# zssjh/stereo-semantic-vo

Measured on AMD Instinct MI355X. Metric: stereo frames/sec on KITTI 00 (full Tracking::Track chain), higher is better.
Workload: dtype u8; 1 GPU; BASELINE configs[2]: synth-kitti00 sequence of 4541 distinct 1241x376 stereo pairs, full Tracking::Track loop per frame (ORB on L and R, sparse stereo, matching passes 1+2, PnP-RANSAC, pose-only LM, map-point lifecycle); ONE sequence per GPU in strict frame order (replicas across GPUs); parallelism=one GPU, resident_pairs_per_gpu=4541, resident_input_bytes_per_gpu=4370984960, frames_tracked=4541, tracker_capacity_flag=0, pnp_samples_through_sequential_fallback=0

## Files before the change

include/svo.h:

```cpp
#ifndef SVO_H
#define SVO_H

#include <stdint.h>

#ifdef __cplusplus
extern "C" {
#endif

#define SVO_ABI_VERSION 8

typedef enum svo_status {
  SVO_OK = 0,
  SVO_E_INVALID = -1,
  SVO_E_NODEVICE = -2,
  SVO_E_NOMEM = -3,
  SVO_E_HIP = -4,
  SVO_E_CAPACITY = -5,
  SVO_E_TIMEOUT = -6
} svo_status;

typedef struct svo_ctx svo_ctx;

typedef struct svo_kp {
  float x, y;
// ... 87 lines not shown
int svo_orb_extract(svo_ctx* ctx, const uint8_t* gray, int stride, svo_kp* kp,
                    uint8_t* desc, int32_t* n);

int svo_debug_pyramid_level(svo_ctx* ctx, int image_slot, int level, uint8_t* out);
int svo_debug_fast_corners(svo_ctx* ctx, int image_slot, int level, int32_t* xy_score,
                           int capacity, int32_t* n);

int svo_stereo_frame(svo_ctx* ctx, const uint8_t* grayL, int strideL, const uint8_t* grayR,
                     int strideR, const svo_camera* cam, svo_kp* kpL, uint8_t* descL,
                     int32_t* nL, float* uR, float* depth);
int svo_stereo_frame_ex(svo_ctx* ctx, const uint8_t* grayL, int strideL, const uint8_t* grayR,
                        int strideR, const svo_camera* cam, svo_kp* kpL, uint8_t* descL,
                        int32_t* nL, float* uR, float* depth, svo_kp* kpR, uint8_t* descR,
                        int32_t* nR);

int svo_debug_stereo_match(svo_ctx* ctx, const uint8_t* grayL, int strideL, const uint8_t* grayR, int strideR,
                           const svo_camera* cam, const svo_kp* kpL, const uint8_t* descL, int nL, const svo_kp* kpR,
                           const uint8_t* descR, int nR, float* uR, float* depth, int32_t* sad);

int svo_disp2depth(svo_ctx* ctx, const float* disp, int count, float bf, float* depth);
int svo_unproject(svo_ctx* ctx, const float* uvz, int n, const svo_camera* cam,
                  const float Rwc[9], const float twc[3], float* xyz);


int svo_descriptor_distance(svo_ctx* ctx, const uint8_t* a, const uint8_t* b, int count,
                            int32_t* dist);

int svo_hamming_argmin(svo_ctx* ctx, const uint8_t* q, int M, const uint8_t* t, int N,
                       const uint8_t* t_mask, int32_t* best_idx, int32_t* best,
                       int32_t* second);

int svo_match_greedy(svo_ctx* ctx, const uint8_t* q, const uint8_t* q_skip, int M,
                     const uint8_t* t, int N, uint8_t* assigned, int max_dist, float ratio,
                     int32_t* best_idx, int32_t* best, int32_t* second, uint8_t* accepted);

int svo_match_greedy_gated(svo_ctx* ctx, const uint8_t* q, const uint8_t* q_skip, int M,
                           const uint8_t* t, int N, uint8_t* assigned, int max_dist, float ratio,
                           const float* q_xy, const float* t_xy, const int32_t* boxes, int n_boxes,
                           const double F[9], int32_t* best_idx, int32_t* best, int32_t* second,
                           uint8_t* accepted, uint8_t* vetoed);

int svo_bf_match(svo_ctx* ctx, const uint8_t* q, int M, const uint8_t* t, int N,
                 int32_t* train_idx, int32_t* dist, uint8_t* keep);

int svo_fundamental_8point(svo_ctx* ctx, const double* pts1, const double* pts2, int n, double F[9]);

int svo_pnp_ransac(svo_ctx* ctx, const double* Xw, const double* obs, int n, const double K[4],
                   const double T_fallback_cw[16], uint64_t rng_state, double T_cw[16],
                   uint8_t* inlier_mask, svo_pnp_stats* stats);

int svo_debug_epnp5(svo_ctx* ctx, const double Xw5[15], const double uv5[10], const double K[4], double R[9],
                    double t[3], double rep_err[3]);

int svo_pose_opt(svo_ctx* ctx, const double* Xw, const double* obs, int n, const double K[4],
                 double T_cw[16], svo_lm_stats* stats);

int svo_track_reset(svo_ctx* ctx, const svo_camera* cam);
int svo_track_frame(svo_ctx* ctx, const uint8_t* grayL, int strideL, const uint8_t* grayR,
                    int strideR, double timestamp, const int32_t* boxes, int n_boxes,
                    svo_track_result* res);

int svo_debug_track_matches(svo_ctx* ctx, int32_t* cur_mp);
int svo_debug_track_gate(svo_ctx* ctx, double F[9], int32_t* n_vetoed);
int svo_debug_track_frames(svo_ctx* ctx, int first, int n, svo_track_debug* out);

int svo_debug_track_depths(svo_ctx* ctx, int frame, svo_kp* kp, float* depth, int32_t* n);

int svo_debug_track_pnp(svo_ctx* ctx, svo_pnp_stats* stats, double T_pnp[16]);

int svo_frontend_batch_dev(svo_ctx* ctx, const uint8_t* d_grayL, const uint8_t* d_grayR,
                           int stride, int B, const svo_camera* cam, svo_kp* d_kpL,
                           uint8_t* d_descL, int32_t* d_nL, float* d_uR, float* d_depth);
int svo_track_batch_dev(svo_ctx* ctx, const uint8_t* d_grayL, const uint8_t* d_grayR,
                        int stride, int B, const svo_boxes_dev* boxes, svo_track_result* d_results);

int svo_track_tail_dev(svo_ctx* ctx, const svo_kp* d_kp, const uint8_t* d_desc, const int32_t* d_n,
                       const float* d_depth, int kp_stride, int B, const svo_boxes_dev* boxes,
                       svo_track_result* d_results);
int svo_track_sharded_dev(svo_ctx* const* ctxs, int G, const uint8_t* const* d_grayL, const uint8_t* const* d_grayR,
                          int stride, int B, const svo_boxes_dev* boxes, svo_track_result* d_results);
int svo_track_batch_host(svo_ctx* ctx, const uint8_t* grayL, const uint8_t* grayR, int stride, int B,
                         const svo_boxes_host* boxes, svo_track_result* results);
int svo_track_sharded_host(svo_ctx* const* ctxs, int G, const uint8_t* grayL, const uint8_t* grayR, int stride, int B,
                           const svo_boxes_host* boxes, svo_track_result* results);
int svo_frontend_batch_host(svo_ctx* ctx, const uint8_t* grayL, const uint8_t* grayR, int stride, int B,
                            const svo_camera* cam, svo_kp* kpL, uint8_t* descL, int32_t* nL, float* uR, float* depth);


int svo_bgr_to_gray(svo_ctx* ctx, const uint8_t* bgr, int width, int height, int bgr_stride, uint8_t* gray, int gray_stride);
int svo_track_frame_bgr(svo_ctx* ctx, const uint8_t* bgrL, int strideL, const uint8_t* bgrR, int strideR, double timestamp,
                        const int32_t* boxes, int n_boxes, svo_track_result* res);
int svo_track_batch_bgr_dev(svo_ctx* ctx, const uint8_t* d_bgrL, const uint8_t* d_bgrR, int stride, int B,
                            const svo_boxes_dev* boxes, svo_track_result* d_results);
int svo_track_batch_bgr_host(svo_ctx* ctx, const uint8_t* bgrL, const uint8_t* bgrR, int stride, int B,
                             const svo_boxes_host* boxes, svo_track_result* results);

int svo_track_overflowed(svo_ctx* ctx, int32_t* flag);
int svo_track_epnp_fallbacks(svo_ctx* ctx, int64_t* count);

int svo_debug_stream_probe(svo_ctx* ctx, int32_t out[2]);

int svo_debug_stream_pipes(svo_ctx* ctx, int32_t out[4]);

int svo_track_multi_reset(svo_ctx* ctx, int n_seq, const svo_camera* cam);
int svo_track_multi_step_dev(svo_ctx* ctx, const uint8_t* d_grayL, const uint8_t* d_grayR, int stride,
                             int n_seq, const svo_boxes_dev* boxes, svo_track_result* d_results);
// ... 203 lines not shown
```

stereo-semantic-vo_amd/__init__.py:

```python
import ctypes as C
import os

import numpy as np

_HERE = os.path.dirname(os.path.abspath(__file__))
LIB_PATH = os.environ.get("SVO_LIB_PATH") or os.path.join(_HERE, "libsvo_hip.so")

KP_DTYPE = np.dtype([("x", "<f4"), ("y", "<f4"), ("size", "<f4"), ("angle", "<f4"),
                     ("response", "<f4"), ("octave", "<i4"), ("class_id", "<i4")])

TRACK_DTYPE = np.dtype([("Tcw", "<f4", (16,)), ("frame_id", "<i4"), ("n_kp", "<i4"),
                        ("n_stereo", "<i4"), ("n_match_pass1", "<i4"), ("n_match_pass2", "<i4"),
                        ("n_pnp_inliers", "<i4"), ("n_lm_edges", "<i4"), ("n_new_mappoints", "<i4"),
                        ("n_local_map", "<i4"), ("lm_iterations", "<i4"), ("reserved", "<i4", (2,))])

TRACK_DEBUG_DTYPE = np.dtype([("match_gid", "<i4", (512,)), ("new_gid", "<i4", (512,)), ("frame_id", "<i4"),
                              ("pnp_best", "<i4"), ("pnp_iterations", "<i4"), ("pnp_inliers", "<i4"), ("pnp_ok", "<i4"),
                              ("active_rows", "<i4", (2,)), ("rounds", "<i4", (2,)), ("resolve_us", "<i4"),
                              ("rt", "<i8", (6,)), ("T_pnp", "<f8", (16,))])

ABI_SYMBOLS = [
    "svo_abi_version", "svo_strerror", "svo_last_error", "svo_create", "svo_destroy", "svo_sync",
    "svo_set_option",
    "svo_stream", "svo_orb_geometry", "svo_orb_extract", "svo_debug_pyramid_level",
    "svo_debug_fast_corners", "svo_stereo_frame", "svo_stereo_frame_ex", "svo_disp2depth",
    "svo_unproject", "svo_descriptor_distance", "svo_hamming_argmin", "svo_match_greedy",
    "svo_match_greedy_gated",
    "svo_bf_match", "svo_pnp_ransac", "svo_debug_epnp5", "svo_pose_opt", "svo_track_reset", "svo_track_frame",
    "svo_debug_track_matches", "svo_debug_track_gate", "svo_debug_track_pnp", "svo_debug_track_frames", "svo_fundamental_8point",
    "svo_frontend_batch_dev", "svo_track_batch_dev", "svo_profile_enable", "svo_profile_reset",
    "svo_profile_get",
    "svo_elas_default_params", "svo_elas_process", "svo_elas_process_ex", "svo_elas_delaunay",
    "svo_ctmf", "svo_track_multi_reset", "svo_track_multi_step_dev", "svo_track_tail_dev", "svo_track_overflowed", "svo_track_epnp_fallbacks", "svo_debug_stream_probe", "svo_debug_stream_pipes", "svo_track_sharded_dev", "svo_elas_batch_dev", "svo_msa_init", "svo_msa_tree", "svo_msa_tree_dp", "svo_msa_wta", "svo_msa_lrcheck", "svo_msa_solve", "svo_msa_batch_dev",
    "svo_create_ex", "svo_stream_mode", "svo_track_batch_host", "svo_track_sharded_host", "svo_frontend_batch_host",
    "svo_bgr_to_gray", "svo_track_frame_bgr", "svo_track_batch_bgr_dev", "svo_track_batch_bgr_host",
    "svo_det_describe", "svo_det_last_error", "svo_det_create", "svo_det_destroy", "svo_det_detect", "svo_det_batch_dev",
    "svo_det_sync", "svo_det_debug_tensor", "svo_det_detect_planar", "svo_det_profile", "svo_det_layer_times",
    "svo_sgbm_default_params", "svo_sgbm_process", "svo_sgbm_batch_dev", "svo_sgbm_debug_volume", "svo_sgbm_filter_speckles",
    "svo_sgbm_default_params_bgr", "svo_sgbm_process_bgr", "svo_sgbm_batch_bgr_dev", "svo_debug_track_depths",
    "svo_sgbm_process_mode", "svo_sgbm_process_bgr_mode", "svo_sgbm_batch_mode_dev", "svo_sgbm_batch_bgr_mode_dev",
    "svo_lk_default_params", "svo_lk_track", "svo_lk_batch_dev", "svo_lk_chain_dev", "svo_lk_debug_level",
    "svo_lk_track_bgr", "svo_lk_batch_bgr_dev", "svo_lk_chain_bgr_dev", "svo_lk_debug_level_bgr",
    "svo_dyn_default_params", "svo_track_dynamic", "svo_track_dynamic_out", "svo_track_multi_step_bgr_dev",
    "svo_debug_stereo_match",
]

CREATE_POOLED_STREAMS = 1
CREATE_TAIL_ALL_CUS = 2


class SvoError(RuntimeError):
    pass


class Camera(C.Structure):
    _fields_ = [("fx", C.c_float), ("fy", C.c_float), ("cx", C.c_float), ("cy", C.c_float),
                ("bf", C.c_float)]


class BoxesDev(C.Structure):
    _fields_ = [("boxes", C.c_void_p), ("n", C.c_void_p), ("stride", C.c_int32)]


def boxes_dev(d_boxes, d_n, stride):
    return BoxesDev(C.c_void_p(int(d_boxes)), C.c_void_p(int(d_n)), int(stride))


def _bx(b):
    return None if b is None else C.byref(b)


class BoxesHost(C.Structure):
    _fields_ = [("boxes", C.c_void_p), ("n", C.c_void_p), ("stride", C.c_int32)]


def boxes_host(boxes, n):
    b = np.ascontiguousarray(boxes, np.int32)
    c = np.ascontiguousarray(n, np.int32)
    r = BoxesHost(b.ctypes.data_as(C.c_void_p), c.ctypes.data_as(C.c_void_p), int(b.shape[1]))
    r._keep = (b, c)
    return r
# ... 202 lines not shown
        sk = None if q_skip is None else _u8(q_skip)
        bi = np.zeros(M, np.int32); b = np.zeros(M, np.int32); s = np.zeros(M, np.int32)
        acc = np.zeros(M, np.uint8)
        self._chk(self.lib.svo_match_greedy(self.h, _p(q), _p(sk), M, _p(t), N, _p(assigned),
                                            int(max_dist), C.c_float(ratio), _p(bi), _p(b), _p(s),
                                            _p(acc)))
        return bi, b, s, acc, assigned

    def match_greedy_gated(self, q, t, assigned, max_dist, ratio, q_xy, t_xy, boxes, F, q_skip=None, vetoed=None):
        q = _u8(q).reshape(-1, 32); t = _u8(t).reshape(-1, 32)
        M, N = len(q), len(t)
        assigned = _u8(assigned).copy()
        sk = None if q_skip is None else _u8(q_skip)
        qxy = np.ascontiguousarray(q_xy, np.float32).reshape(-1, 2)
        txy = np.ascontiguousarray(t_xy, np.float32).reshape(-1, 2)
        if len(qxy) != M or len(txy) != N:
            raise SvoError("match_greedy_gated: q_xy / t_xy must hold one point per descriptor row")
        bx = None if boxes is None or len(boxes) == 0 else np.ascontiguousarray(boxes, np.int32).reshape(-1, 4)
        nb = 0 if bx is None else len(bx)
        Fm = np.ascontiguousarray(F, np.float64).reshape(9)
        bi = np.zeros(M, np.int32); b = np.zeros(M, np.int32); s = np.zeros(M, np.int32)
        acc = np.zeros(M, np.uint8)
        vet = np.zeros(M, np.uint8) if vetoed is None else vetoed
        if vet.dtype != np.uint8 or vet.shape != (M,) or not vet.flags.c_contiguous:
            raise SvoError("match_greedy_gated: vetoed must be a contiguous uint8 array of M entries")
        self._chk(self.lib.svo_match_greedy_gated(self.h, _p(q), _p(sk), M, _p(t), N, _p(assigned), int(max_dist),
                                                  C.c_float(ratio), _p(qxy), _p(txy), _p(bx), nb, _p(Fm), _p(bi), _p(b),
                                                  _p(s), _p(acc), _p(vet)))
        return bi, b, s, acc, assigned, vet

    def bf_match(self, q, t):
        q = _u8(q).reshape(-1, 32); t = _u8(t).reshape(-1, 32)
        M, N = len(q), len(t)
        ti = np.zeros(M, np.int32); d = np.zeros(M, np.int32); keep = np.zeros(M, np.uint8)
        self._chk(self.lib.svo_bf_match(self.h, _p(q), M, _p(t), N, _p(ti), _p(d), _p(keep)))
        return ti, d, keep

    def pnp_ransac(self, Xw, obs, K, T_fallback, rng_state=0):
        Xw = np.ascontiguousarray(Xw, np.float64).reshape(-1, 3)
        obs = np.ascontiguousarray(obs, np.float64).reshape(-1, 2)
        K = np.ascontiguousarray(K, np.float64)
        Tp = np.ascontiguousarray(T_fallback, np.float64).reshape(16)
        T = np.zeros(16); mask = np.zeros(max(len(Xw), 1), np.uint8); st = PnpStats()
        self._chk(self.lib.svo_pnp_ransac(self.h, _p(Xw), _p(obs), len(Xw), _p(K), _p(Tp),
                                          C.c_uint64(rng_state), _p(T), _p(mask), C.byref(st)))
        return T.reshape(4, 4), mask[:len(Xw)], st

    def debug_epnp5(self, Xw5, uv5, K):
        Xw5 = np.ascontiguousarray(Xw5, np.float64).reshape(15); uv5 = np.ascontiguousarray(uv5, np.float64).reshape(10)
        K = np.ascontiguousarray(K, np.float64); R = np.zeros(9); t = np.zeros(3); rep = np.zeros(3)
        self._chk(self.lib.svo_debug_epnp5(self.h, _p(Xw5), _p(uv5), _p(K), _p(R), _p(t), _p(rep)))
        return R.reshape(3, 3), t, rep

    def pose_opt(self, Xw, obs, K, T):
        Xw = np.ascontiguousarray(Xw, np.float64).reshape(-1, 3)
        obs = np.ascontiguousarray(obs, np.float64).reshape(-1, 2)
        K = np.ascontiguousarray(K, np.float64)
        T = np.ascontiguousarray(T, np.float64).reshape(16).copy()
        st = LmStats()
        self._chk(self.lib.svo_pose_opt(self.h, _p(Xw), _p(obs), len(Xw), _p(K), _p(T), C.byref(st)))
        return T.reshape(4, 4), st

    def track_reset(self, cam):
        self._chk(self.lib.svo_track_reset(self.h, C.byref(cam)))

    def track_frame(self, grayL, grayR, timestamp=0.0, boxes=None):
        grayL = _u8(grayL); grayR = _u8(grayR)
        res = np.zeros(1, TRACK_DTYPE)
        bx = None if boxes is None or len(boxes) == 0 else np.ascontiguousarray(boxes, np.int32)
        nb = 0 if bx is None else len(bx)
        self._chk(self.lib.svo_track_frame(self.h, _p(grayL), self.W, _p(grayR), self.W,
                                           C.c_double(timestamp), _p(bx), nb, _p(res)))
        return res[0]

    def bgr_to_gray(self, bgr):
        a = _u8(bgr)
        H, W = a.shape[:2]
        out = np.zeros((H, W), np.uint8)
        self._chk(self.lib.svo_bgr_to_gray(self.h, _p(a), W, H, 3 * W, _p(out), W))
        return out

    def track_frame_bgr(self, bgrL, bgrR, timestamp=0.0, boxes=None):
        bgrL = _u8(bgrL); bgrR = _u8(bgrR)
        res = np.zeros(1, TRACK_DTYPE)
        bx = None if boxes is None or len(boxes) == 0 else np.ascontiguousarray(boxes, np.int32)
        nb = 0 if bx is None else len(bx)
        self._chk(self.lib.svo_track_frame_bgr(self.h, _p(bgrL), 3 * self.W, _p(bgrR), 3 * self.W,
                                               C.c_double(timestamp), _p(bx), nb, _p(res)))
        return res[0]

    def track_batch_bgr_dev(self, d_bgrL, d_bgrR, stride, B, d_results, boxes=None):
        self._chk(self.lib.svo_track_batch_bgr_dev(self.h, _p(d_bgrL), _p(d_bgrR), int(stride), int(B), _bx(boxes),
                                                   _p(d_results)))

    def track_batch_bgr_host(self, bgrL, bgrR, stride, B, results, boxes=None):
        self._chk(self.lib.svo_track_batch_bgr_host(self.h, _p(bgrL), _p(bgrR), int(stride), int(B), _bx(boxes), _p(results)))

    def debug_track_gate(self):
        F = np.zeros(9); n = C.c_int32(0)
        self._chk(self.lib.svo_debug_track_gate(self.h, _p(F), C.byref(n)))
        return F.reshape(3, 3), n.value

    def fundamental_8point(self, pts1, pts2):
        pts1 = np.ascontiguousarray(pts1, np.float64).reshape(-1, 2)
        pts2 = np.ascontiguousarray(pts2, np.float64).reshape(-1, 2)
        F = np.zeros(9)
# ... 526 lines not shown
```

stereo-semantic-vo_amd/csrc/svo_api.hip:

```cpp
#include <math.h>
#include <string.h>

#include <algorithm>
#include <thread>
#include <stdio.h>
#include <stdlib.h>

#include <chrono>
#include <functional>
#include <initializer_list>
#include "svo_internal.h"

struct PendingEvt { int entry; hipEvent_t a, b; };

struct SvoProfState {
  std::vector<PendingEvt> pending;
  std::vector<hipEvent_t> pool;
};
static SvoProfState* prof_state(svo_ctx* ctx) {
  if (!ctx->prof_impl) ctx->prof_impl = new SvoProfState();
  return reinterpret_cast<SvoProfState*>(ctx->prof_impl);
}
static void prof_resolve(svo_ctx* ctx) {
  SvoProfState* ps = prof_state(ctx);
// ... 810 lines not shown
  hipSetDevice(ctx->device);
  Bump bm{ctx};
  double* dX = bm.take<double>(3 * (size_t)std::max(n, 1));
  double* dO = bm.take<double>(2 * (size_t)std::max(n, 1));
  double* dK = bm.take<double>(4);
  double* dTp = bm.take<double>(16);
  double* dT = bm.take<double>(16);
  uint8_t* dM = bm.take<uint8_t>(std::max(n, 1));
  svo_pnp_stats* dS = bm.take<svo_pnp_stats>(1);
  uint16_t* dSub = bm.take<uint16_t>(512);
  void* dHyp = bm.take<uint8_t>(svo_pnp_hyp_bytes());
  if (!bm.ok()) return SVO_E_CAPACITY;
  if (n > 0) { H2D(dX, Xw, 24 * (size_t)n); H2D(dO, obs, 16 * (size_t)n); }
  H2D(dK, K, 32);
  H2D(dTp, T_fallback_cw, 128);
  const uint16_t* sub = ctx->d_pnp_subsets + (size_t)std::min(n, 512) * 500;
  uint16_t hsub[500];
  if (rng_state != 0 && rng_state != ~0ull) {
    svo_pnp_subsets(rng_state, n, hsub);
    H2D(dSub, hsub, sizeof hsub);
    SVO_HIP(ctx, hipStreamSynchronize(ctx->stream));
    sub = dSub;
  }
  int rc = svo_launch_pnp(ctx, dX, dO, n, dK, dTp, sub, dHyp, dT, dM, dS);
  if (rc) return rc;
  D2H(T_cw, dT, 128);
  if (inlier_mask && n > 0) D2H(inlier_mask, dM, n);
  if (stats) D2H(stats, dS, sizeof(svo_pnp_stats));
  SVO_HIP(ctx, hipStreamSynchronize(ctx->stream));
  return SVO_OK;
}

extern "C" int svo_debug_epnp5(svo_ctx* ctx, const double Xw5[15], const double uv5[10], const double K[4], double R[9],
                               double t[3], double rep_err[3]) {
  if (!ctx || !Xw5 || !uv5 || !K || !R || !t) return SVO_E_INVALID;
  hipSetDevice(ctx->device);
  Bump bm{ctx};
  double* dX = bm.take<double>(15); double* dU = bm.take<double>(10); double* dK = bm.take<double>(4);
  double* dO = bm.take<double>(24);
  if (!bm.ok()) return SVO_E_CAPACITY;
  H2D(dX, Xw5, 120); H2D(dU, uv5, 80); H2D(dK, K, 32);
  const char* reps_env = getenv("SVO_EPNP_REPS");
  int rc = svo_launch_epnp5_probe(ctx, dX, dU, dK, dO, reps_env ? atoi(reps_env) : 1);
  if (rc) return rc;
  double o[24];
  D2H(o, dO, sizeof o);
  SVO_HIP(ctx, hipStreamSynchronize(ctx->stream));
  memcpy(R, o, 72); memcpy(t, o + 9, 24);
  if (rep_err) memcpy(rep_err, o + 13, 24);
  if (getenv("SVO_EPNP_STAMPS")) fprintf(stderr, "epnp5 cycles: setup+MtM %.0f, eigen %.0f (%d sweeps), L/rho %.0f, branches %.0f (initial betas %.0f, Gauss-Newton %.0f, to the last SVD %.0f)\n", o[16], o[17], (int)o[20], o[18], o[19], o[21], o[22], o[23]);
  return o[12] != 0.0 ? SVO_OK : SVO_E_INVALID;
}

static int frontend_slice(svo_ctx* ctx, hipStream_t st, const uint8_t* d_grayL, const uint8_t* d_grayR, int stride, int p0, int b,
                          const svo_camera* cam, svo_kp* d_kpL, uint8_t* d_descL, int32_t* d_nL, float* d_uR, float* d_depth) {
  const size_t K = ctx->max_kp, img = (size_t)ctx->g.H * stride;
  const SvoFeBufs fb = svo_fe_own(ctx).at(ctx->g, K, 2 * (size_t)p0, p0);
  int rc = svo_launch_orb(ctx, st, fb, d_grayL + p0 * img, d_grayR + p0 * img, stride, b, 2 * b);
  if (rc == SVO_OK) rc = svo_launch_stereo(ctx, st, fb, d_grayL + p0 * img, d_grayR + p0 * img, stride, b, cam);
  if (rc == SVO_OK) {
    auto d2d = [&](void* dst, const void* src, size_t bytes) {
      if (dst && hipMemcpyAsync(dst, src, bytes, hipMemcpyDeviceToDevice, st) != hipSuccess) rc = SVO_E_HIP;
    };
    d2d(d_kpL ? d_kpL + (size_t)p0 * K : nullptr, fb.kp, sizeof(svo_kp) * K * b);
    d2d(d_descL ? d_descL + (size_t)p0 * K * 32 : nullptr, fb.desc, 32 * K * b);
    d2d(d_nL ? d_nL + p0 : nullptr, fb.nkp, 4 * (size_t)b);
    d2d(d_uR ? d_uR + (size_t)p0 * K : nullptr, fb.uR, 4 * K * b);
    d2d(d_depth ? d_depth + (size_t)p0 * K : nullptr, fb.depth, 4 * K * b);
  }
  return rc;
}

int svo_frontend_nslices(const svo_ctx* ctx, int B) {
  const int ns = std::min(ctx->opt_frontend_overlap, B / 8);
  return (ns < 2 || ctx->profiling) ? 1 : ns;
}

extern "C" int svo_frontend_batch_dev(svo_ctx* ctx, const uint8_t* d_grayL, const uint8_t* d_grayR,
                                      int stride, int B, const svo_camera* cam, svo_kp* d_kpL,
                                      uint8_t* d_descL, int32_t* d_nL, float* d_uR,
                                      float* d_depth) {
  if (!ctx || !d_grayL || !d_grayR || !cam || B < 1 || stride < ctx->g.W) return SVO_E_INVALID;
  if (B > ctx->max_batch) return SVO_E_CAPACITY;
  hipSetDevice(ctx->device);
  { const int rcq = svo_track_quiesce(ctx); if (rcq) return rcq; }
  const int ns = svo_frontend_nslices(ctx, B);
  if (ns < 2)
    return frontend_slice(ctx, ctx->stream, d_grayL, d_grayR, stride, 0, B, cam, d_kpL, d_descL, d_nL, d_uR, d_depth);
  while ((int)ctx->fe_streams.size() < ns - 1) {
    hipStream_t st = nullptr;
    hipEvent_t e;
    {
      int attempts = 0, percent = 0;
      const int rcp = svo_pick_stream(ctx, [](hipStream_t* s) { return svo_stream_create(s, 0); },
                                      {ctx->stream, ctx->fe_streams.empty() ? nullptr : ctx->fe_streams.back()}, &st, &attempts, &percent,
                                      {ctx->stream, ctx->fe_streams.empty() ? nullptr : ctx->fe_streams.back()},
                                      {ctx->stream, ctx->fe_streams.empty() ? nullptr : ctx->fe_streams.back()});
      if (rcp) return rcp;
    }
    ctx->fe_streams.push_back(st);
    SVO_HIP(ctx, hipEventCreateWithFlags(&e, hipEventDisableTiming));
    ctx->fe_events.push_back(e);
  }
  if (!ctx->ev_frontend) SVO_HIP(ctx, hipEventCreateWithFlags(&ctx->ev_frontend, hipEventDisableTiming));
  SVO_HIP(ctx, hipEventRecord(ctx->ev_frontend, ctx->stream));
  int rc = SVO_OK;
// ... 223 lines not shown
```

stereo-semantic-vo_amd/csrc/svo_epnp_ord_dev.h:

```cpp
#pragma once
#ifndef HIP_INCLUDE_HIP_HIP_RUNTIME_H
#include <hip/hip_runtime.h>
#endif
#include <stdint.h>

#include "svo_epnp_exact_dev.h"

namespace epnp_ord {

#define EO_FN __device__ __forceinline__
typedef double d2 __attribute__((ext_vector_type(2)));

#include "svo_epnp_ord_tab.h"
#include "svo_epnp_ord_asm.h"

#define EO_SYNC()                                         \
  do {                                                    \
    __builtin_amdgcn_fence(__ATOMIC_ACQ_REL, "wavefront"); \
    __builtin_amdgcn_wave_barrier();                      \
  } while (0)

struct Lds {
  alignas(16) double jr[16 * 16];
  alignas(16) double xch[16][4][4];
// ... 377 lines not shown
        const double delta = (gamma - beta) * 0.5;
        sn = xsqrt(xdiv(delta, gamma));
        c = xdiv(p, gamma * sn * 2);
      } else {
        c = xsqrt(xdiv(gamma + beta, gamma * 2));
        sn = xdiv(p, gamma * c * 2);
      }
      const double se = is_j ? -sn : sn;
      const double n0 = c * x0 + se * y0, n1 = c * x1 + se * y1, n2 = c * x2 + se * y2;
      const double Wn = colsum<12>(n0 * n0, n1 * n1, n2 * n2, g);
      EO_SYNC();
      if (rot) {
        x0 = n0; x1 = n1; x2 = n2; W = Wn;
        chg |= 1u << sw;
        mine[0] = x0; mine[1] = x1; mine[2] = x2;
        S.xw[r] = W;
      }
    }
    EO_SYNC();
    const bool closes = active && (e & 0x80u) != 0;
    if (__any(closes)) {
      const int sc = sbase + (int)((e >> 8) & 3);
      const unsigned long long bal = __ballot(closes && ((chg >> (sc & 31)) & 1u));
      if (closes && (sc >= 29 || ((unsigned)bal & pm) == 0u)) active = false;
    }
    tt = tn; tp = tpn; sbase = sbn; e = en;
    ++nsteps;
  }
  if (lane == 0) S.sweeps = 1000000 + nsteps;
  EO_SYNC();
}

typedef __attribute__((address_space(3))) double lds_double;
__device__ __attribute__((noinline)) void svd_small_seq(Lds& S, double* jW, int M, int n, int base, int p) {
  double w[6];
  epnp_exact::jacobi_svd((lds_double*)jW, (lds_double*)&S.jr[base * 16], 16, w, (lds_double*)&S.jr[base * 16 + M], 16, M, n, n);
  for (int i = 0; i < n; ++i) {
    S.sw[p][i] = w[i];
    S.srow[p][i] = base + i;
    S.jr[(base + i) * 16 + 15] = w[i];
  }
  S.flag |= 2; S.why |= 8;
}

__device__ __attribute__((noinline)) void svd12_finish_seq(Lds& S, epnp_exact::Work& xw) {
  for (int i = 0; i < 12; ++i)
    for (int k = 0; k < 12; ++k) xw.ut[i * 12 + k] = S.xch[i][k & 3][k >> 2];
  epnp_exact::jacobi_svd_finish((lds_double*)xw.jW, (lds_double*)xw.ut, 12, xw.d, (lds_double*)nullptr, 0, 12, 12, 12);
  for (int q = 0; q < 4; ++q)
    for (int k = 0; k < 12; ++k) S.ut4[q][k] = xw.ut[(11 - q) * 12 + k];
  S.flag |= 2; S.why |= 4;
}

EO_FN void gauss_newton(Lds& S, int cand, int col, bool owner, const double* L, const double* rho, double* betas) {
  for (int it = 0; it < 5; ++it) {
    double A[6][4], b[6];
    {
      const int i = col < 6 ? col : 0;
      const double* rl = L + 10 * i;
      double* g = S.gn[cand][i];
      const double a0 = 2 * rl[0] * betas[0] + rl[1] * betas[1] + rl[3] * betas[2] + rl[6] * betas[3];
      const double a1 = rl[1] * betas[0] + 2 * rl[2] * betas[1] + rl[4] * betas[2] + rl[7] * betas[3];
      const double a2 = rl[3] * betas[0] + rl[4] * betas[1] + 2 * rl[5] * betas[2] + rl[8] * betas[3];
      const double a3 = rl[6] * betas[0] + rl[7] * betas[1] + rl[8] * betas[2] + 2 * rl[9] * betas[3];
      const double bi = rho[i] - (rl[0] * betas[0] * betas[0] + rl[1] * betas[0] * betas[1] + rl[2] * betas[1] * betas[1] +
                                  rl[3] * betas[0] * betas[2] + rl[4] * betas[1] * betas[2] + rl[5] * betas[2] * betas[2] +
                                  rl[6] * betas[0] * betas[3] + rl[7] * betas[1] * betas[3] + rl[8] * betas[2] * betas[3] +
                                  rl[9] * betas[3] * betas[3]);
      if (owner && col < 6) { g[0] = a0; g[1] = a1; g[2] = a2; g[3] = a3; g[4] = bi; }
    }
    EO_SYNC();
#pragma unroll
    for (int i = 0; i < 6; ++i) {
      const double* g = S.gn[cand][i];
      A[i][0] = g[0]; A[i][1] = g[1]; A[i][2] = g[2]; A[i][3] = g[3]; b[i] = g[4];
    }
    EO_SYNC();
    double A1[4], A2[4], x[4] = {0, 0, 0, 0};
    bool alive = true;
#pragma unroll
    for (int k = 0; k < 4; ++k) {
      double eta = fabs(A[k][k]);
#pragma unroll
      for (int i = k + 1; i < 6; ++i) {
        const double elt = fabs(A[i - 1][k]);
        if (eta < elt) eta = elt;
      }
      if (eta == 0) alive = false;
      const double inv_eta = 1. / eta;
      double sum2 = 0.0;
#pragma unroll
      for (int i = k; i < 6; ++i) {
        A[i][k] *= inv_eta;
        sum2 += A[i][k] * A[i][k];
      }
      double sigma = xsqrt(sum2);
      if (A[k][k] < 0) sigma = -sigma;
      A[k][k] += sigma;
      A1[k] = sigma * A[k][k];
      A2[k] = -eta * sigma;
#pragma unroll
      for (int j = k + 1; j < 4; ++j) {
        double sum = 0;
#pragma unroll
        for (int i = k; i < 6; ++i) sum += A[i][k] * A[i][j];
        const double tau = sum / A1[k];
#pragma unroll
        for (int i = k; i < 6; ++i) A[i][j] -= tau * A[i][k];
      }
    }
#pragma unroll
    for (int j = 0; j < 4; ++j) {
      double tau = 0;
#pragma unroll
      for (int i = j; i < 6; ++i) tau += A[i][j] * b[i];
      tau /= A1[j];
#pragma unroll
      for (int i = j; i < 6; ++i) b[i] -= tau * A[i][j];
    }
    x[3] = b[3] / A2[3];
#pragma unroll
    for (int i = 2; i >= 0; --i) {
      double sum = 0;
#pragma unroll
      for (int j = i + 1; j < 4; ++j) sum += A[i][j] * x[j];
      x[i] = (b[i] - sum) / A2[i];
    }
#pragma unroll
    for (int i = 0; i < 4; ++i) betas[i] += alive ? x[i] : 0.0;
  }
}

EO_FN double dot3(const double* a, const double* b) { return a[0] * b[0] + a[1] * b[1] + a[2] * b[2]; }

EO_FN bool solve5_wave(Lds& S, epnp_exact::Work& xw, const double* K, double* R_out, double* t_out, double* rep, bool force_seq = false) {
  const int lane = threadIdx.x & 63, slot = lane >> 4, col = lane & 15, r16 = lane & 15;
  const double fu = K[0], fv = K[1], uc = K[2], vc = K[3];
  if (lane == 0) { S.flag = force_seq ? 1 : 0; S.why = force_seq ? 16 : 0; S.stamp[0] = clock64(); }
  load_tables(S, lane);
  EO_SYNC();
  if (lane < 3) {
    double c = 0;
    for (int i = 0; i < 5; i++) c += S.pws[3 * i + lane];
    S.cws[lane] = c / 5;
  }
  EO_SYNC();
  auto load_pw0 = [&]() {
    if (lane < 9) {
      const int a = lane / 3, b = lane % 3;
      const double ca = S.cws[a], cb = S.cws[b];
      double s = 0;
      for (int i = 0; i < 5; ++i) s += (S.pws[3 * i + a] - ca) * (S.pws[3 * i + b] - cb);
      S.jr[b * 16 + a] = s;
    } else if (lane < 18) {
      const int r = (lane - 9) / 3, k = (lane - 9) % 3;
      S.jr[r * 16 + 3 + k] = r == k ? 1.0 : 0.0;
    } else if (lane < 36) {
      S.jr[((lane - 18) / 6) * 16 + 6 + (lane - 18) % 6] = 0.0;
    }
    EO_SYNC();
  };
  load_pw0();
  EO_PROF3_BEGIN();
  unsigned long long ex = jacobi_rows<3>(S, r16 < 3 ? 3 : 0, r16 < 3 ? 0 : r16, lane);
  EO_PROF3_END(0);
  unsigned long long bd = svd_rank(S, slot == 0 ? 3 : 0, 0, 0, lane);
  if (ex | bd) {
    load_pw0();
    if (lane == 0) svd_small_seq(S, xw.jW, 3, 3, 0, 0);
    EO_SYNC();
  }
  if (lane < 9) {
    const int i = 1 + lane / 3, j = lane % 3;
    const double k = xsqrt(S.sw[0][i - 1] / 5);
    S.cws[3 * i + j] = S.cws[j] + k * S.jr[S.srow[0][i - 1] * 16 + j];
  }
  EO_SYNC();
  auto load_cc = [&]() {
    if (lane < 9) {
      const int r = lane / 3, k = lane % 3;
      S.jr[r * 16 + k] = S.cws[3 * (r + 1) + k] - S.cws[k];
    } else if (lane < 18) {
      const int r = (lane - 9) / 3, k = (lane - 9) % 3;
      S.jr[r * 16 + 3 + k] = r == k ? 1.0 : 0.0;
// ... 286 lines not shown
```

stereo-semantic-vo_amd/csrc/svo_internal.h:

```cpp
#pragma once
#include <hip/hip_runtime.h>
#include <stdint.h>

#include <chrono>
#include <functional>
#include <initializer_list>
#include <string>
#include <atomic>
#include <vector>

#include "../../include/svo.h"

#define SVO_NLEVELS 8
#define SVO_EDGE 31
#define SVO_FAST_THR 20
#define SVO_HALF_PATCH 15
#define SVO_CAP1 1024
#define SVO_QMAX 128
#define SVO_DESC_BYTES 32

#define FAST_TW 120
#define FAST_TH 30

struct SvoGeom {
// ... 168 lines not shown
  std::vector<SvoProfileEntry> prof;
  void* prof_impl = nullptr;
};

#define SVO_HIP(ctx, expr)                                                        \
  do {                                                                            \
    hipError_t _e = (expr);                                                       \
    if (_e != hipSuccess) {                                                       \
      (ctx)->last_error = std::string(#expr) + ": " + hipGetErrorString(_e);      \
      return SVO_E_HIP;                                                           \
    }                                                                             \
  } while (0)

static inline hipError_t svo_memcpy_sync(svo_ctx* ctx, void* dst, const void* src, size_t bytes, hipMemcpyKind kind) {
  hipError_t e = hipMemcpyAsync(dst, src, bytes, kind, ctx->stream);
  if (e == hipSuccess) e = hipStreamSynchronize(ctx->stream);
  return e;
}

static inline SvoFeBufs svo_fe_own(const svo_ctx* ctx) {
  SvoFeBufs b;
  b.pyr = ctx->d_pyr; b.corners = ctx->d_corners; b.counters = ctx->d_counters; b.hist = ctx->d_hist;
  b.sel = ctx->d_sel; b.selcnt = ctx->d_selcnt;
  b.kp = ctx->d_kp; b.desc = ctx->d_desc; b.nkp = ctx->d_nkp; b.uR = ctx->d_uR; b.depth = ctx->d_depth; b.sad = ctx->d_sad;
  return b;
}

int svo_launch_orb(svo_ctx* ctx, hipStream_t st, const SvoFeBufs& b, const uint8_t* d_grayL, const uint8_t* d_grayR,
                   int stride, int B, int nimg);
int svo_launch_stereo(svo_ctx* ctx, hipStream_t st, const SvoFeBufs& b, const uint8_t* d_grayL, const uint8_t* d_grayR,
                      int stride, int B, const svo_camera* cam);
int svo_launch_descriptor_distance(svo_ctx* ctx, const uint8_t* a, const uint8_t* b, int count,
                                   int32_t* dist);
int svo_launch_hamming_argmin(svo_ctx* ctx, const uint8_t* q, int M, const uint8_t* t, int N,
                              const uint8_t* mask, int32_t* idx, int32_t* best, int32_t* second);
int svo_launch_match_greedy(svo_ctx* ctx, const uint8_t* q, const uint8_t* q_skip, int M,
                            const uint8_t* t, int N, uint8_t* assigned, int max_dist, float ratio,
                            int32_t* idx, int32_t* best, int32_t* second, uint8_t* accepted,
                            const float* q_xy = nullptr, const float* t_xy = nullptr,
                            const int32_t* boxes = nullptr, int n_boxes = 0, const double* F = nullptr,
                            uint8_t* vetoed = nullptr);
int svo_launch_bf_match(svo_ctx* ctx, const uint8_t* q, int M, const uint8_t* t, int N,
                        int32_t* train_idx, int32_t* dist, uint8_t* keep);
int svo_launch_bf_match_dev(svo_ctx* ctx, const uint8_t* q, const int* M_ptr, const uint8_t* t,
                            const int* N_ptr, int Mmax, int32_t* train_idx, int32_t* dist,
                            uint8_t* keep, int32_t* gmin);
int svo_launch_pose_opt(svo_ctx* ctx, const double* Xw, const double* obs, int n, const double* K,
                        double* T, svo_lm_stats* stats);
int svo_launch_pnp(svo_ctx* ctx, const double* Xw, const double* obs, int n, const double* K,
                   const double* Tfallback, const uint16_t* subset, void* hyp, double* T, uint8_t* mask,
                   svo_pnp_stats* stats);
size_t svo_pnp_hyp_bytes();
int svo_launch_epnp5_probe(svo_ctx* ctx, const double* X5, const double* u5, const double* K, double* Rt, int reps);
void svo_pnp_subsets(uint64_t state, int n, uint16_t* out );
int svo_pose_lds_optin(svo_ctx* ctx);
template <typename T>
__host__ __device__ inline T* svo_byte_offset(T* p, size_t bytes) {
  return p ? reinterpret_cast<T*>(reinterpret_cast<uintptr_t>(p) + bytes) : p;
}
hipError_t svo_stream_create(hipStream_t* st, int role);
int svo_stream_burst(svo_ctx* ctx);
struct MsaBfsRec { int32_t cpos, meta, ppos, node; };
int svo_msa_tree_rec(const uint8_t* m_img3, const double* r_gra, const double* c_gra, int width, int height, MsaBfsRec* rec,
                     std::vector<int32_t>* level_ptr, int* maxw, int32_t* root);
int svo_track_quiesce(svo_ctx* ctx, bool shard_too = true);
int svo_shard_quiesce(svo_ctx* ctx);
int svo_track_check_timeout(svo_ctx* ctx);
int svo_hostfeed_flush(svo_ctx* ctx);
void svo_hostfeed_release(svo_ctx* ctx);
int svo_pick_stream(svo_ctx* ctx, const std::function<hipError_t(hipStream_t*)>& make, std::initializer_list<hipStream_t> others, hipStream_t* out,
                    int* attempts, int* percent, std::initializer_list<hipStream_t> holds_up = {}, std::initializer_list<hipStream_t> held_up_by = {});
int svo_probe_block_percent(hipStream_t blocker, hipStream_t victim);
int svo_track_fe_batch_stream(svo_ctx* ctx);
int svo_elas_batch_dev_hooked(svo_ctx* ctx, hipStream_t s, const uint8_t* d_L, const uint8_t* d_R, int stride, int W, int H, int B,
                              const svo_elas_params* params, float* d_D1, float* d_D2, int32_t* produced,
                              int (*hook)(void*, int, int), void* user);
struct SvoBgrSrc {
  const uint8_t* L = nullptr;
  const uint8_t* R = nullptr;
  int stride = 0;
  bool convert = false;
  const hipEvent_t* wait = nullptr;
  int n_wait = 0;
  hipEvent_t done = nullptr;
};
int svo_track_batch_fed(svo_ctx* ctx, const uint8_t* d_grayL, const uint8_t* d_grayR, int stride, int B,
                        const svo_boxes_dev* boxes, svo_track_result* d_results, const hipEvent_t* pair_ready,
                        const SvoBgrSrc* bgr = nullptr);
int svo_track_frame_staged(svo_ctx* ctx, const int32_t* boxes, int n_boxes, svo_track_result* res, const uint8_t* d_bgrL,
                           const uint8_t* d_bgrR, int bgr_pitch);
void svo_launch_bgr2gray(hipStream_t st, const uint8_t* bgr, int bgr_stride, size_t bgr_frame, uint8_t* gray, int gray_pitch,
                         size_t gray_frame, int W, int H, int n);
void svo_colour_release(svo_ctx* ctx);
int svo_track_sharded_fed(svo_ctx* const* ctxs, int G, const uint8_t* const* d_grayL, const uint8_t* const* d_grayR, int stride, int B,
                          const svo_boxes_dev* boxes, svo_track_result* d_results, const hipEvent_t* const* pair_ready);
hipError_t svo_stream_create_masked(hipStream_t* st, int device, int percent);
int svo_frontend_nslices(const svo_ctx* ctx, int B);
int svo_launch_disp2depth(svo_ctx* ctx, const float* disp, int count, float bf, float* depth);
int svo_launch_unproject(svo_ctx* ctx, const float* uvz, int n, const svo_camera* cam,
                         const float* Rwc, const float* twc, float* xyz);

extern "C" void svo_elas_release(svo_ctx* ctx);
void svo_msa_release(svo_ctx* ctx);
void svo_sgbm_release(svo_ctx* ctx);
void svo_lk_release(svo_ctx* ctx);
struct LkArena {
// ... 75 lines not shown
```

stereo-semantic-vo_amd/csrc/svo_pose.hip:

```cpp
#include "svo_pose_dev.h"

extern __shared__ __attribute__((aligned(16))) unsigned char pose_smem[];

__global__ __launch_bounds__(256) void k_pose_opt(const double* __restrict__ Xw,
                                                  const double* __restrict__ obs, int n,
                                                  const double* __restrict__ Kp, double* T,
                                                  svo_lm_stats* stats, const int* n_ptr,
                                                  int round_in_f32, int use_mfma, size_t seq_stride) {
  if (blockIdx.y) {
    const size_t off = (size_t)blockIdx.y * seq_stride;
    Xw = svo_byte_offset(Xw, off); obs = svo_byte_offset(obs, off); Kp = svo_byte_offset(Kp, off);
    T = svo_byte_offset(T, off); stats = svo_byte_offset(stats, off); n_ptr = svo_byte_offset(n_ptr, off);
  }
  if (n_ptr) n = *n_ptr;
  PoseLds& L = *reinterpret_cast<PoseLds*>(pose_smem);
  pose_opt_block(L, Xw, obs, n, Kp, T, stats, round_in_f32, use_mfma);
}

struct PnpHypLds {
  double Xw[PNP_MAXN * 3], uv[PNP_MAXN * 2];
  EpnpWaveLds ws[4];
};

__global__ __launch_bounds__(256) void k_pnp_hyp(const double* __restrict__ Xw, const double* __restrict__ obs, int n,
// ... 50 lines not shown
    }
  } else {
    if (inlier_mask)
      for (int e = tid; e < n; e += 256) inlier_mask[e] = 0;
    if (tid < 16) T[tid] = Tfallback[tid];
  }
  if (tid == 0 && stats) {
    stats->n_points = n; stats->n_inliers = best >= 0 ? s_good : 0; stats->best_hypothesis = best;
    stats->ok = best >= 0 ? 1 : 0; stats->iterations = s_iters;
  }
}

__global__ __launch_bounds__(256) void k_epnp5_probe(const double* X5, const double* u5, const double* Kp, double* Rt, int reps) {
  __shared__ EpnpWaveLds wsv[4];
  EpnpWaveLds& ws = wsv[threadIdx.x >> 6];
  const int lane = threadIdx.x & 63;
  double K[4] = {Kp[0], Kp[1], Kp[2], Kp[3]}, R[9], t[3];
  if (lane < 15) ws.x5[lane] = X5[lane];
  if (lane < 10) ws.u5[lane] = u5[lane];
  bool ok = false;
  for (int rep = 0; rep < reps; ++rep) ok = epnp5_wave(ws, K, R, t);
  if (threadIdx.x == 0 && blockIdx.x == 0) {
    for (int i = 0; i < 9; ++i) Rt[i] = R[i];
    Rt[9] = t[0]; Rt[10] = t[1]; Rt[11] = t[2]; Rt[12] = ok ? 1.0 : 0.0;
    for (int b = 0; b < 3; ++b) Rt[13 + b] = ws.out[b][12];
    for (int b = 0; b < 4; ++b) Rt[16 + b] = (double)(ws.stamp[b + 1] - ws.stamp[b]);
    Rt[20] = ws.sweeps;
    Rt[21] = (double)(ws.stamp[5] - ws.stamp[3]); Rt[22] = (double)(ws.stamp[6] - ws.stamp[5]); Rt[23] = (double)(ws.stamp[7] - ws.stamp[6]);
  }
}
__global__ __launch_bounds__(64) void k_epnp5_probe_exact(const double* X5, const double* u5, const double* Kp, double* Rt) {
  __shared__ epnp_exact::Work W;
  if (threadIdx.x != 0 || blockIdx.x != 0) return;
  double K[4] = {Kp[0], Kp[1], Kp[2], Kp[3]};
  const bool ok = epnp_exact::solve5(W, X5, u5, K, Rt, Rt + 9, Rt + 13);
  Rt[12] = ok ? 1.0 : 0.0;
  for (int b = 16; b < 24; ++b) Rt[b] = 0.0;
}
__global__ __launch_bounds__(64) void k_epnp5_probe_ord(const double* X5, const double* u5, const double* Kp, double* Rt, int force_seq) {
  __shared__ PnpOrdLds L;
  const int lane = threadIdx.x;
  if (lane < 15) L.S.pws[lane] = X5[lane];
  if (lane < 10) L.S.us[lane] = u5[lane];
  double K[4] = {Kp[0], Kp[1], Kp[2], Kp[3]}, R[9], t[3], rep[3];
  const bool ok = epnp_ord::solve5_wave(L.S, L.W, K, R, t, rep, force_seq != 0);
  if (lane == 0 && blockIdx.x == 0) {
    for (int i = 0; i < 9; ++i) Rt[i] = R[i];
    Rt[9] = t[0]; Rt[10] = t[1]; Rt[11] = t[2]; Rt[12] = ok ? 1.0 : 0.0;
    for (int b = 0; b < 3; ++b) Rt[13 + b] = rep[b];
    for (int b = 0; b < 7; ++b) Rt[16 + b] = (double)(L.S.stamp[b + 1] - L.S.stamp[b]);
    Rt[23] = (double)L.S.flag;
  }
}
int svo_launch_epnp5_probe(svo_ctx* ctx, const double* X5, const double* u5, const double* K, double* Rt, int reps) {
  if (ctx->opt_epnp_exact == 2) {
    hipLaunchKernelGGL(k_epnp5_probe_ord, dim3(1), dim3(64), 0, ctx->stream, X5, u5, K, Rt, ctx->opt_epnp_force_seq);
    SVO_HIP(ctx, hipGetLastError());
    return SVO_OK;
  }
  if (ctx->opt_epnp_exact) {
    hipLaunchKernelGGL(k_epnp5_probe_exact, dim3(1), dim3(64), 0, ctx->stream, X5, u5, K, Rt);
    SVO_HIP(ctx, hipGetLastError());
    return SVO_OK;
  }
  const char* wv = getenv("SVO_EPNP_WAVES");
  const char* gv = getenv("SVO_EPNP_GRID");
  const int waves = wv ? std::min(std::max(atoi(wv), 1), 4) : 1, grid = gv ? std::max(atoi(gv), 1) : 1;
  hipLaunchKernelGGL(k_epnp5_probe, dim3(grid), dim3(64 * waves), 0, ctx->stream, X5, u5, K, Rt, reps < 1 ? 1 : reps);
  SVO_HIP(ctx, hipGetLastError());
  return SVO_OK;
}

int svo_pose_lds_optin(svo_ctx* ctx) {
  if (ctx->pose_lds_state == 0) {
    bool ok = hipFuncSetAttribute(reinterpret_cast<const void*>(k_pose_opt), hipFuncAttributeMaxDynamicSharedMemorySize,
                                  (int)sizeof(PoseLds)) == hipSuccess;
    ok = ok && hipFuncSetAttribute(reinterpret_cast<const void*>(k_pnp_hyp), hipFuncAttributeMaxDynamicSharedMemorySize,
                                   (int)sizeof(PnpHypLds)) == hipSuccess;
    ctx->pose_lds_state = ok ? 1 : -1;
    if (!ok) ctx->last_error = std::string("hipFuncSetAttribute(pose kernels): ") + hipGetErrorString(hipGetLastError());
  }
  return ctx->pose_lds_state > 0 ? SVO_OK : SVO_E_HIP;
}

void svo_pnp_subsets(uint64_t state, int n, uint16_t* out ) {
  if (!state) state = ~0ull;
  auto next = [&]() -> unsigned {
    state = (uint64_t)(unsigned)state * 4164903690U + (unsigned)(state >> 32);
    return (unsigned)state;
  };
  for (int k = 0; k < PNP_HYP; ++k) {
    int idx[5];
    for (int i = 0; i < 5; ++i) {
      if (n <= 5) { idx[i] = i < n ? i : 0; continue; }
      for (;;) {
        const int c = idx[i] = (int)(next() % (unsigned)n);
        int j = 0;
        for (; j < i; ++j)
          if (c == idx[j]) break;
        if (j == i) break;
      }
    }
    for (int i = 0; i < 5; ++i) out[5 * k + i] = (uint16_t)idx[i];
  }
}

// ... 32 lines not shown
```

Measured before the change: 10320 stereo frames/s.

## Parallelize EPnP Gauss-Newton Householder QR across lanes via DPP broadcasts

Replaces the per-thread sequential Gauss-Newton beta refinement in the ordered EPnP solver with a lane-parallel version. Each lane builds one row of the 6x4 Jacobian, and a Householder QR runs with four lanes per candidate, each owning one column, exchanging values through DPP quad broadcasts. The old scalar path is kept behind EO_GN_SCALAR, and a debug probe kernel and API entry point are added for checking the result. The goal is to shorten the serial latency of the EPnP hypothesis solve, at the cost of extra LDS syncs and possible small floating-point ordering differences.

```diff
diff --git a/include/svo.h b/include/svo.h
--- a/include/svo.h
+++ b/include/svo.h
@@ -163,6 +163,9 @@
 int svo_debug_epnp5(svo_ctx* ctx, const double Xw5[15], const double uv5[10], const double K[4], double R[9],
                     double t[3], double rep_err[3]);
 
+int svo_debug_epnp_gn(svo_ctx* ctx, const double L[60], const double rho[6], const double betas_in[12],
+                      double betas_out[12]);
+
 int svo_pose_opt(svo_ctx* ctx, const double* Xw, const double* obs, int n, const double K[4],
                  double T_cw[16], svo_lm_stats* stats);
 
diff --git a/stereo-semantic-vo_amd/__init__.py b/stereo-semantic-vo_amd/__init__.py
--- a/stereo-semantic-vo_amd/__init__.py
+++ b/stereo-semantic-vo_amd/__init__.py
@@ -26,7 +26,7 @@
     "svo_debug_fast_corners", "svo_stereo_frame", "svo_stereo_frame_ex", "svo_disp2depth",
     "svo_unproject", "svo_descriptor_distance", "svo_hamming_argmin", "svo_match_greedy",
     "svo_match_greedy_gated",
-    "svo_bf_match", "svo_pnp_ransac", "svo_debug_epnp5", "svo_pose_opt", "svo_track_reset", "svo_track_frame",
+    "svo_bf_match", "svo_pnp_ransac", "svo_debug_epnp5", "svo_debug_epnp_gn", "svo_pose_opt", "svo_track_reset", "svo_track_frame",
     "svo_debug_track_matches", "svo_debug_track_gate", "svo_debug_track_pnp", "svo_debug_track_frames", "svo_fundamental_8point",
     "svo_frontend_batch_dev", "svo_track_batch_dev", "svo_profile_enable", "svo_profile_reset",
     "svo_profile_get",
@@ -335,6 +335,12 @@
         self._chk(self.lib.svo_debug_epnp5(self.h, _p(Xw5), _p(uv5), _p(K), _p(R), _p(t), _p(rep)))
         return R.reshape(3, 3), t, rep
 
+    def debug_epnp_gn(self, L, rho, betas):
+        L = np.ascontiguousarray(L, np.float64).reshape(60); rho = np.ascontiguousarray(rho, np.float64).reshape(6)
+        betas = np.ascontiguousarray(betas, np.float64).reshape(12); out = np.zeros(12)
+        self._chk(self.lib.svo_debug_epnp_gn(self.h, _p(L), _p(rho), _p(betas), _p(out)))
+        return out.reshape(3, 4)
+
     def pose_opt(self, Xw, obs, K, T):
         Xw = np.ascontiguousarray(Xw, np.float64).reshape(-1, 3)
         obs = np.ascontiguousarray(obs, np.float64).reshape(-1, 2)
diff --git a/stereo-semantic-vo_amd/csrc/svo_api.hip b/stereo-semantic-vo_amd/csrc/svo_api.hip
--- a/stereo-semantic-vo_amd/csrc/svo_api.hip
+++ b/stereo-semantic-vo_amd/csrc/svo_api.hip
@@ -886,6 +886,20 @@
   return o[12] != 0.0 ? SVO_OK : SVO_E_INVALID;
 }
 
+extern "C" int svo_debug_epnp_gn(svo_ctx* ctx, const double L[60], const double rho[6], const double betas_in[12], double betas_out[12]) {
+  if (!ctx || !L || !rho || !betas_in || !betas_out) return SVO_E_INVALID;
+  hipSetDevice(ctx->device);
+  Bump bm{ctx};
+  double* dL = bm.take<double>(60); double* dR = bm.take<double>(6); double* dB = bm.take<double>(12); double* dO = bm.take<double>(12);
+  if (!bm.ok()) return SVO_E_CAPACITY;
+  H2D(dL, L, 480); H2D(dR, rho, 48); H2D(dB, betas_in, 96);
+  int rc = svo_launch_epnp_gn_probe(ctx, dL, dR, dB, dO);
+  if (rc) return rc;
+  D2H(betas_out, dO, 96);
+  SVO_HIP(ctx, hipStreamSynchronize(ctx->stream));
+  return SVO_OK;
+}
+
 static int frontend_slice(svo_ctx* ctx, hipStream_t st, const uint8_t* d_grayL, const uint8_t* d_grayR, int stride, int p0, int b,
                           const svo_camera* cam, svo_kp* d_kpL, uint8_t* d_descL, int32_t* d_nL, float* d_uR, float* d_depth) {
   const size_t K = ctx->max_kp, img = (size_t)ctx->g.H * stride;
diff --git a/stereo-semantic-vo_amd/csrc/svo_epnp_ord_dev.h b/stereo-semantic-vo_amd/csrc/svo_epnp_ord_dev.h
--- a/stereo-semantic-vo_amd/csrc/svo_epnp_ord_dev.h
+++ b/stereo-semantic-vo_amd/csrc/svo_epnp_ord_dev.h
@@ -453,6 +453,95 @@
   S.flag |= 2; S.why |= 4;
 }
 
+#ifndef EO_GN_SCALAR
+template <int Q>
+EO_FN double quad_bcast(double v) {
+  return __longlong_as_double(__builtin_amdgcn_mov_dpp(__double_as_longlong(v), 0x150 + Q, 0xf, 0xf, false));
+}
+template <int K>
+EO_FN void gn_step(int q, double (&p)[6], double (&o)[6], double (&R)[4][4], double* A2, bool& alive) {
+  double eta = fabs(p[K]);
+#pragma unroll
+  for (int i = K + 1; i < 6; ++i) {
+    const double elt = fabs(p[i - 1]);
+    if (eta < elt) eta = elt;
+  }
+  if (eta == 0) alive = false;
+  const double inv_eta = 1. / eta;
+  double sum2 = 0.0;
+#pragma unroll
+  for (int i = K; i < 6; ++i) {
+    p[i] *= inv_eta;
+    sum2 += p[i] * p[i];
+  }
+  double sigma = xsqrt(sum2);
+  if (p[K] < 0) sigma = -sigma;
+  p[K] += sigma;
+  const double A1 = sigma * p[K];
+  A2[K] = -eta * sigma;
+  if (K == 0 || q >= K) {
+    double sum = 0;
+#pragma unroll
+    for (int i = K; i < 6; ++i) sum += p[i] * o[i];
+    const double tau = sum / A1;
+#pragma unroll
+    for (int i = K; i < 6; ++i) o[i] -= tau * p[i];
+  }
+  if (K < 1) R[K][1] = quad_bcast<0>(o[K]);
+  if (K < 2) R[K][2] = quad_bcast<1>(o[K]);
+  if (K < 3) R[K][3] = quad_bcast<2>(o[K]);
+  R[K][0] = quad_bcast<3>(o[K]);
+  if (K < 3) {
+#pragma unroll
+    for (int i = K + 1; i < 6; ++i) p[i] = quad_bcast<K>(o[i]);
+  }
+}
+EO_FN void gauss_newton(Lds& S, int cand, int col, bool owner, const double* L, const double* rho, double* betas) {
+  const int q = col & 3;
+#pragma unroll 1
+  for (int it = 0; it < 5; ++it) {
+    {
+      const int i = col < 6 ? col : 0;
+      const double* rl = L + 10 * i;
+      double (*g)[6] = S.gn[cand];
+      const double a0 = 2 * rl[0] * betas[0] + rl[1] * betas[1] + rl[3] * betas[2] + rl[6] * betas[3];
+      const double a1 = rl[1] * betas[0] + 2 * rl[2] * betas[1] + rl[4] * betas[2] + rl[7] * betas[3];
+      const double a2 = rl[3] * betas[0] + rl[4] * betas[1] + 2 * rl[5] * betas[2] + rl[8] * betas[3];
+      const double a3 = rl[6] * betas[0] + rl[7] * betas[1] + rl[8] * betas[2] + 2 * rl[9] * betas[3];
+      const double bi = rho[i] - (rl[0] * betas[0] * betas[0] + rl[1] * betas[0] * betas[1] + rl[2] * betas[1] * betas[1] +
+                                  rl[3] * betas[0] * betas[2] + rl[4] * betas[1] * betas[2] + rl[5] * betas[2] * betas[2] +
+                                  rl[6] * betas[0] * betas[3] + rl[7] * betas[1] * betas[3] + rl[8] * betas[2] * betas[3] +
+                                  rl[9] * betas[3] * betas[3]);
+      if (owner && col < 6) { g[0][i] = a0; g[1][i] = a1; g[2][i] = a2; g[3][i] = a3; g[4][i] = bi; }
+    }
+    EO_SYNC();
+    double p[6], o[6];
+    {
+      const double* g0 = S.gn[cand][0];
+      const double* gq = S.gn[cand][q + 1];
+#pragma unroll
+      for (int i = 0; i < 6; ++i) { p[i] = g0[i]; o[i] = gq[i]; }
+    }
+    EO_SYNC();
+    double R[4][4], A2[4], x[4];
+    bool alive = true;
+    gn_step<0>(q, p, o, R, A2, alive);
+    gn_step<1>(q, p, o, R, A2, alive);
+    gn_step<2>(q, p, o, R, A2, alive);
+    gn_step<3>(q, p, o, R, A2, alive);
+    x[3] = R[3][0] / A2[3];
+#pragma unroll
+    for (int i = 2; i >= 0; --i) {
+      double sum = 0;
+#pragma unroll
+      for (int j = i + 1; j < 4; ++j) sum += R[i][j] * x[j];
+      x[i] = (R[i][0] - sum) / A2[i];
+    }
+#pragma unroll
+    for (int i = 0; i < 4; ++i) betas[i] += alive ? x[i] : 0.0;
+  }
+}
+#else
 EO_FN void gauss_newton(Lds& S, int cand, int col, bool owner, const double* L, const double* rho, double* betas) {
   for (int it = 0; it < 5; ++it) {
     double A[6][4], b[6];
@@ -531,6 +620,7 @@
     for (int i = 0; i < 4; ++i) betas[i] += alive ? x[i] : 0.0;
   }
 }
+#endif
 
 EO_FN double dot3(const double* a, const double* b) { return a[0] * b[0] + a[1] * b[1] + a[2] * b[2]; }
 
diff --git a/stereo-semantic-vo_amd/csrc/svo_internal.h b/stereo-semantic-vo_amd/csrc/svo_internal.h
--- a/stereo-semantic-vo_amd/csrc/svo_internal.h
+++ b/stereo-semantic-vo_amd/csrc/svo_internal.h
@@ -244,6 +244,7 @@
                    svo_pnp_stats* stats);
 size_t svo_pnp_hyp_bytes();
 int svo_launch_epnp5_probe(svo_ctx* ctx, const double* X5, const double* u5, const double* K, double* Rt, int reps);
+int svo_launch_epnp_gn_probe(svo_ctx* ctx, const double* L60, const double* rho6, const double* betas_in, double* betas_out);
 void svo_pnp_subsets(uint64_t state, int n, uint16_t* out );
 int svo_pose_lds_optin(svo_ctx* ctx);
 template <typename T>
diff --git a/stereo-semantic-vo_amd/csrc/svo_pose.hip b/stereo-semantic-vo_amd/csrc/svo_pose.hip
--- a/stereo-semantic-vo_amd/csrc/svo_pose.hip
+++ b/stereo-semantic-vo_amd/csrc/svo_pose.hip
@@ -126,6 +126,23 @@
     Rt[23] = (double)L.S.flag;
   }
 }
+__global__ __launch_bounds__(64) void k_epnp_gn_probe(const double* L60, const double* rho6, const double* betas_in, double* betas_out) {
+  __shared__ epnp_ord::Lds S;
+  const int lane = threadIdx.x, slot = lane >> 4, col = lane & 15, cand = slot < 3 ? slot : 0;
+  if (lane < 60) S.L[lane] = L60[lane];
+  EO_SYNC();
+  double rho[6], betas[4];
+  for (int k = 0; k < 6; ++k) rho[k] = rho6[k];
+  for (int k = 0; k < 4; ++k) betas[k] = betas_in[4 * cand + k];
+  epnp_ord::gauss_newton(S, cand, col, slot < 3, S.L, rho, betas);
+  if (slot < 3 && col < 4 && blockIdx.x == 0) betas_out[4 * cand + col] = col == 0 ? betas[0] : (col == 1 ? betas[1] : (col == 2 ? betas[2] : betas[3]));
+}
+int svo_launch_epnp_gn_probe(svo_ctx* ctx, const double* L60, const double* rho6, const double* betas_in, double* betas_out) {
+  hipLaunchKernelGGL(k_epnp_gn_probe, dim3(1), dim3(64), 0, ctx->stream, L60, rho6, betas_in, betas_out);
+  SVO_HIP(ctx, hipGetLastError());
+  return SVO_OK;
+}
+
 int svo_launch_epnp5_probe(svo_ctx* ctx, const double* X5, const double* u5, const double* K, double* Rt, int reps) {
   if (ctx->opt_epnp_exact == 2) {
     hipLaunchKernelGGL(k_epnp5_probe_ord, dim3(1), dim3(64), 0, ctx->stream, X5, u5, K, Rt, ctx->opt_epnp_force_seq);
```

After: 10490 stereo frames/s (median of 6 runs). 1.02x the previous value.
